# HandBrake/HandBrake

Measured on AMD Instinct MI355X. Metric: filtered frames/sec, 1080p YUV420p NLMeans+decomb chain, higher is better.
Workload: dtype u8 (f32 NLMeans weights, 16-bit fixed-point scaler as zimg, sharpen mix = the reference's f64 expression, as one f32 multiply where init proves that equal); 1 GPU; BASELINE configs[3]: decomb(31, EEDI2 bob) -> nlmeans medium -> cropscale lanczos 1920x1080 -> 3840x2160 -> lapsharp, 1080i YUV420P 8-bit in, inputs resident in HBM; input=1920x1080, output=3840x2160, streams_per_gpu=1, content=interlaced, stream_frames=48, stage_streams=2, parallelism=1 GPU(s) x 1 independent stream(s), device=AMD Radeon Graphics (gfx950:sramecc+:xnack-, 256 CUs)

## Files before the change

### handbrake_amd/csrc/nlmeans.hip

```cpp
#include "hbhip_internal.h"

#include <algorithm>
#include <type_traits>
#include <unordered_map>

namespace {

constexpr int PX = 4;
constexpr int RY = 8;
constexpr int TXN = 32;
constexpr int TYN = 8;
constexpr int TH = TYN * RY;
constexpr int NLM_BORDER = 16;
#ifndef NLM16_SYM_PAIRS
#define NLM16_SYM_PAIRS 3
#endif

struct alignas(16) NlmJob
{
    const uint8_t *frame[HBHIP_NLMEANS_FRAMES_MAX];
    int            fpitch[HBHIP_NLMEANS_FRAMES_MAX];
    const uint8_t *frame_pre[HBHIP_NLMEANS_FRAMES_MAX];
    int            ppitch[HBHIP_NLMEANS_FRAMES_MAX];
    const uint8_t *src_pre;
    int            src_pre_pitch;
    uint8_t       *dst;
    const float   *exptable;
    double         origin_tune;
    float          wft;
    int            diff_max;
    int            diff_cap;
    uint32_t       imul4;
    int            ishift;
    int            w, h, dst_pitch;
    int            nframes, r_half;
    int            tiles_x, tile_start;
};

__global__ void job_table_kernel(uint4 *__restrict__ dst, const uint4 *__restrict__ src, int n16)
{
    const int i = blockIdx.x * blockDim.x + threadIdx.x;
    if (i < n16) dst[i] = src[i];
}

struct __attribute__((packed, aligned(1))) u32_unaligned { uint32_t v; };
typedef float f2 __attribute__((ext_vector_type(2)));

__device__ __forceinline__ int reflect(int x, int n)
{
    x = x < 0 ? -1 - x : x;
    x = x >= n ? 2 * n - 1 - x : x;
    return min(max(x, 0), n - 1);
}

__device__ __forceinline__ uint32_t byte_of(uint32_t v, int k) { return (v >> (8 * k)) & 0xffu; }

constexpr int LTXA = TXN - 2;
constexpr int LTW = LTXA * PX;

__device__ __forceinline__ void load_tile_p(uint32_t *lds, int pitch, int dwords, int rows,
                                            const uint8_t *__restrict__ plane, int src_pitch,
                                            int w, int h, int x0, int y0)
{
    int tid = threadIdx.x;
    asm volatile("" : "+v"(tid));
    const int rpp = (TXN * TYN) / dwords;
    const int r0 = (int)(((float)tid + 0.5f) * (1.0f / (float)dwords));
    const int c = tid - r0 * dwords;
    if (r0 >= rpp) return;
    const int x = x0 + 4 * c;
    const bool whole = x >= 0 && x + 3 < w;
    const int o0 = reflect(x, w), o1 = reflect(x + 1, w), o2 = reflect(x + 2, w), o3 = reflect(x + 3, w);
    uint32_t *out = lds + r0 * pitch + c;
    if (y0 >= 0 && y0 + rows <= h && x0 >= 0 && x0 + 4 * dwords <= w)
    {
        const uint8_t *ptr = plane + (size_t)(y0 + r0) * src_pitch + x;
        const size_t step = (size_t)rpp * src_pitch;
#pragma nounroll
        for (int r = r0; r < rows; r += rpp, out += rpp * pitch, ptr += step)
            *out = reinterpret_cast<const u32_unaligned *>(ptr)->v;
        return;
    }
#pragma nounroll
    for (int r = r0; r < rows; r += rpp, out += rpp * pitch)
    {
        const uint8_t *row = plane + (size_t)reflect(y0 + r, h) * src_pitch;
        uint32_t v;
        if (whole)
            v = reinterpret_cast<const u32_unaligned *>(row + x)->v;
        else
            v = (uint32_t)row[o0] | ((uint32_t)row[o1] << 8) | ((uint32_t)row[o2] << 16) | ((uint32_t)row[o3] << 24);
        *out = v;
    }
}

__device__ __forceinline__ uint32_t from_lane_below(uint32_t x)
{
    return (uint32_t)__builtin_amdgcn_update_dpp(0, (int)x, 0x138 , 0xf, 0xf, false);
}
__device__ __forceinline__ uint32_t from_lane_above(uint32_t x)
{
    return (uint32_t)__builtin_amdgcn_update_dpp(0, (int)x, 0x130 , 0xf, 0xf, false);
}

static bool nlm_no_static_lds(const void *kernel)
{
    hipFuncAttributes a;
    memset(&a, 0, sizeof(a));
    if (hipFuncGetAttributes(&a, kernel) != hipSuccess) { (void)hipGetLastError(); return false; }
    return a.sharedSizeBytes == 0;
}

template <int N, int FAST, int CPD, bool PRE>
__global__ __launch_bounds__(TXN * TYN, 3) void nlmeans_lanes_kernel(const NlmJob *__restrict__ jobs, int njobs,
                                                                     int cmp_rows, int rq)
{
    constexpr int NH = N / 2;
    constexpr int ROWS = RY + N - 1;
    constexpr bool INTIDX = FAST >= 2;
    constexpr bool SYM = FAST == 3 && !PRE;
    static_assert(FAST != 3 || N <= 7, "the pairs' sharing reads a neighbouring lane's edge pixel: patch sizes up to 7");
    constexpr int ST_ROWS = RY + 1, ST_SLOT = ST_ROWS * TXN * TYN;
    static_assert(NH <= PX, "patch must not reach past the adjacent lane");
    static_assert(CPD % 8 == 4, "the two tile rows of a wave must sit 32 banks apart");

    extern __shared__ uint32_t smem[];
    const int tile_dwords = CPD * cmp_rows + 4;
    float *s_exp = reinterpret_cast<float *>(smem);
    uint32_t *s_t0 = smem + 128;
    uint32_t *s_tc = s_t0 + tile_dwords;
    uint32_t *s_r0 = PRE ? s_tc + tile_dwords : s_t0;
    uint32_t *s_rc = PRE ? s_r0 + tile_dwords : s_tc;
    uint32_t *s_stash = s_tc;

    int j = 0;
    for (int hi = njobs - 1; j < hi;)
    {
        const int mid = (j + hi + 1) >> 1;
        if ((int)blockIdx.x >= jobs[mid].tile_start) j = mid; else hi = mid - 1;
    }
    const NlmJob &job = jobs[j];
    const int tile = blockIdx.x - job.tile_start;
    const int tile_y = tile / job.tiles_x;
    int tile_x = tile - tile_y * job.tiles_x;
    if (HBHIP_GRID_ROTATE && (job.tiles_x & 1) == 0) { tile_x += tile_y % job.tiles_x; if (tile_x >= job.tiles_x) tile_x -= job.tiles_x; }
    const int tx0 = tile_x * LTW, ty0 = tile_y * TH;
    const int w = job.w, h = job.h;
    const int RH = job.r_half;

    const int tx = threadIdx.x & (TXN - 1);
    const int ty = threadIdx.x / TXN;

    typedef __attribute__((address_space(3))) const float lds_cfloat;
    __builtin_assume(!INTIDX || reinterpret_cast<uintptr_t>((__attribute__((address_space(3))) uint32_t *)smem) == 0);
    if (threadIdx.x < 128) s_exp[threadIdx.x] = job.exptable[threadIdx.x];
    if (PRE)
    {
        load_tile_p(s_t0, CPD, CPD, cmp_rows, job.src_pre, job.src_pre_pitch, w, h,
                    tx0 - PX - 4 * rq, ty0 - NH - RH);
        load_tile_p(s_r0, CPD, CPD, cmp_rows, job.frame[0], job.fpitch[0], w, h,
                    tx0 - PX - 4 * rq, ty0 - NH - RH);
    }
    else
    {
        load_tile_p(s_t0, CPD, CPD, cmp_rows, job.frame[0], job.fpitch[0], w, h,
                    tx0 - PX - 4 * rq, ty0 - NH - RH);
    }
    const int own_off = (ty * RY + RH) * CPD + tx + rq;
    const uint32_t *own = s_t0 + own_off;
    const uint32_t *own_raw = s_r0 + own_off;

    f2 aw[RY][PX / 2], ap[RY][PX / 2];
#pragma unroll
    for (int o = 0; o < RY; o++)
#pragma unroll
        for (int p = 0; p < PX / 2; p++) { aw[o][p] = f2{0.f, 0.f}; ap[o][p] = f2{0.f, 0.f}; }
    const f2 wft2 = {job.wft, job.wft};

    const float wft = job.wft;
    const int diff_max = job.diff_max;
    const int diff_cap = job.diff_cap;
    const uint32_t imul4 = job.imul4;
    const double origin_tune = job.origin_tune;
    const bool wave_live = ty0 + (ty & ~1) * RY < h;

    for (int f = 0; f < job.nframes; f++)
    {
        if (PRE || f > 0)
        {
            __syncthreads();
            if (PRE)
            {
                load_tile_p(s_tc, CPD, CPD, cmp_rows, job.frame_pre[f], job.ppitch[f], w, h,
                            tx0 - PX - 4 * rq, ty0 - NH - RH);
                if (f > 0)
                    load_tile_p(s_rc, CPD, CPD, cmp_rows, job.frame[f], job.fpitch[f], w, h,
                                tx0 - PX - 4 * rq, ty0 - NH - RH);
            }
            else
            {
                load_tile_p(s_tc, CPD, CPD, cmp_rows, job.frame[f], job.fpitch[f], w, h,
                            tx0 - PX - 4 * rq, ty0 - NH - RH);
            }
        }
        __syncthreads();
        if (!wave_live) continue;
        const uint32_t *cmp_tile = (PRE || f > 0) ? s_tc : s_t0;
        const uint32_t *pix_tile = f > 0 ? s_rc : s_r0;

        auto displacement = [&](auto f0c, int dy, int dx) __attribute__((always_inline))
        {
            constexpr bool F0 = decltype(f0c)::value;
            {
                if (f == 0 && dx == 0 && dy == 0)
                {
#pragma unroll
                    for (int o = 0; o < RY; o++)
                    {
                        const uint32_t cpx = own_raw[(o + NH) * CPD];
#pragma unroll
                        for (int p = 0; p < PX; p++)
                        {
                            aw[o][p / 2][p & 1] = (float)((double)aw[o][p / 2][p & 1] + origin_tune);
                            ap[o][p / 2][p & 1] = (float)((double)ap[o][p / 2][p & 1] + origin_tune * (double)(int)byte_of(cpx, p));
                            __builtin_amdgcn_sched_barrier(0);
                        }
                    }
                    return;
                }

                const int s = dx + 4 * rq;
                const int sh = s & 3;
                if (SYM && F0 && (dy > 0 || (dy == 0 && dx > 0)))
                {
                    const uint32_t *st = s_stash + ((-dy + 1) * 3 + (-dx + 1)) * ST_SLOT + dy * (TXN * TYN) + (int)threadIdx.x;
                    const uint32_t *prow = pix_tile + (ty * RY + dy + RH + NH) * CPD + tx + (s >> 2);
#pragma unroll
                    for (int o = 0; o < RY; o++)
                    {
                        const uint32_t w0 = st[o * (TXN * TYN)];
                        uint32_t id4 = w0;
                        if (dx > 0) id4 = __builtin_amdgcn_alignbyte(st[o * (TXN * TYN) + 1], w0, 1);
                        else if (dx < 0) id4 = __builtin_amdgcn_alignbyte(w0, st[o * (TXN * TYN) - 1], 3);
                        const uint32_t pix = __builtin_amdgcn_alignbyte(prow[o * CPD + 1], prow[o * CPD], sh);
                        const uint32_t o0 = (id4 << 2) & 0x1fcu, o1 = (id4 >> 6) & 0x1fcu, o2 = (id4 >> 14) & 0x1fcu, o3 = (id4 >> 22) & 0x1fcu;
                        const f2 wa = {*reinterpret_cast<lds_cfloat *>(o0), *reinterpret_cast<lds_cfloat *>(o1)};
                        const f2 wb = {*reinterpret_cast<lds_cfloat *>(o2), *reinterpret_cast<lds_cfloat *>(o3)};
                        const f2 pa = {(float)(int)byte_of(pix, 0), (float)(int)byte_of(pix, 1)};
                        const f2 pb = {(float)(int)byte_of(pix, 2), (float)(int)byte_of(pix, 3)};
                        aw[o][0] += wa; ap[o][0] += wa * pa;
                        aw[o][1] += wb; ap[o][1] += wb * pb;
                    }
                    return;
                }
                constexpr bool stash_on = SYM && F0;
                const bool extra_row = stash_on && dy < 0;
                uint32_t *stw = s_stash + ((dy + 1) * 3 + (dx + 1)) * ST_SLOT + (int)threadIdx.x;
                const uint32_t *srow = own;
                const uint32_t *crow = cmp_tile + (ty * RY + dy + RH) * CPD + tx + (s >> 2);

                uint32_t C[PX], hist[RY - 1 + (SYM ? 1 : 0)][PX], v[PX];
                uint32_t centre[NH + 1];
                uint32_t pixq = 0;
                f2 wq[PX / 2];
                const uint32_t *prow = pix_tile + (ty * RY + dy + RH + NH) * CPD + tx + (s >> 2);
#pragma unroll
                for (int q = 0; q < PX; q++) C[q] = 0;

                uint32_t a_n = srow[0], b_n0 = crow[0], b_n1 = crow[1];
#pragma unroll
                for (int i = 0; i < ROWS + (SYM ? 1 : 0); i++)
                {
                    if (!(SYM && i == ROWS) || extra_row)
                    {
                    const uint32_t a = a_n;
                    const uint32_t bw = __builtin_amdgcn_alignbyte(b_n1, b_n0, sh);
                    if (i + 1 < ROWS || (SYM && i + 1 == ROWS && extra_row))
                    {
                        a_n = srow[(i + 1) * CPD];
                        b_n0 = crow[(i + 1) * CPD];
                        b_n1 = crow[(i + 1) * CPD + 1];
                    }
                    if (!PRE) centre[i % (NH + 1)] = bw;
#pragma unroll
                    for (int q = 0; q < PX; q++)
                    {
                        const int d = (int)byte_of(a, q) - (int)byte_of(bw, q);
                        C[q] += (uint32_t)(d * d);
                        if (i < RY - 1 + (SYM ? 1 : 0)) hist[i][q] = C[q];
                    }
                    if (i >= N - 1)
                    {
                        const int o = i - (N - 1);
                        uint32_t V[PX], pre[PX + 1], suf[PX + 1];
#pragma unroll
                        for (int q = 0; q < PX; q++) V[q] = o > 0 ? C[q] - hist[o > 0 ? o - 1 : 0][q] : C[q];
                        pre[0] = 0; suf[0] = 0;
#pragma unroll
                        for (int q = 0; q < PX; q++)
                        {
                            pre[q + 1] = pre[q] + V[q];
                            suf[q + 1] = suf[q] + V[PX - 1 - q];
                        }
#pragma unroll
                        for (int p = 0; p < PX; p++)
                        {
                            const int lo = p - NH, hi = p + NH;
// ... 35 lines not shown
                        {
                            const int o = i - (N - 1);
                            pixq = __builtin_amdgcn_alignbyte(prow[o * CPD + 1], prow[o * CPD], sh);
                        }
                        else
                            pixq = centre[(i - NH) % (NH + 1)];
#pragma unroll
                        for (int pp = 0; pp < PX / 2; pp++)
                        {
                            if (INTIDX)
                                wq[pp] = f2{*reinterpret_cast<lds_cfloat *>(offs[2 * pp]), *reinterpret_cast<lds_cfloat *>(offs[2 * pp + 1])};
                            else
                            {
                                int idx[2];
                                if (FAST == 1)
                                {
                                    const f2 fd = {(float)(int)min(v[2 * pp], (uint32_t)diff_cap),
                                                   (float)(int)min(v[2 * pp + 1], (uint32_t)diff_cap)};
                                    const f2 fi = fd * wft2;
                                    idx[0] = (int)fi.x;
                                    idx[1] = (int)fi.y;
                                }
                                else
                                {
#pragma unroll
                                    for (int e = 0; e < 2; e++)
                                    {
                                        const int diff = (int)v[2 * pp + e];
                                        int ix = (int)((float)diff * wft);
                                        ix = diff < diff_max ? ix : 127;
                                        idx[e] = min(ix, 127);
                                    }
                                }
                                wq[pp] = f2{s_exp[idx[0]], s_exp[idx[1]]};
                            }
                        }
                        }
                    }
                    }
                    __builtin_amdgcn_sched_barrier(0);
                }
                {
                    const uint32_t pix = pixq;
#pragma unroll
                    for (int pp = 0; pp < PX / 2; pp++)
                    {
                        const f2 pv = {(float)(int)byte_of(pix, 2 * pp), (float)(int)byte_of(pix, 2 * pp + 1)};
                        aw[RY - 1][pp] += wq[pp];
                        ap[RY - 1][pp] += wq[pp] * pv;
                    }
                }
            }
        };
        for (int dy = -RH; dy <= RH; dy++)
            for (int dx = -RH; dx <= RH; dx++)
            {
                if (SYM && f == 0) displacement(std::true_type{}, dy, dx);
                else displacement(std::false_type{}, dy, dx);
            }
    }

    const int x = tx0 + (tx - 1) * PX;
    if (tx == 0 || tx == TXN - 1 || x >= w) return;
#pragma unroll
    for (int o = 0; o < RY; o++)
    {
        const int y = ty0 + ty * RY + o;
        if (y >= h) break;
        uint32_t packed = 0;
        const uint32_t cpx = own_raw[(o + NH) * CPD];
#pragma unroll
        for (int p = 0; p < PX; p++)
        {
            const float q = ap[o][p / 2][p & 1] / aw[o][p / 2][p & 1];
            uint32_t r = (uint32_t)(int)q & 0xffu;
            if (r == 0) r = byte_of(cpx, p);
            packed |= r << (8 * p);
            __builtin_amdgcn_sched_barrier(0);
        }
        uint8_t *out = job.dst + (size_t)y * job.dst_pitch + x;
        if (x + 3 < w)
        {
            *reinterpret_cast<uint32_t *>(out) = packed;
        }
        else
        {
            for (int p = 0; p < PX && x + p < w; p++) out[p] = (uint8_t)(packed >> (8 * p));
        }
    }
}

__device__ __forceinline__ void load_tile16(uint32_t *lds, int pitch, int dwords, int rows,
                                            const uint8_t *__restrict__ plane, int src_pitch_bytes,
                                            int w, int h, int x0, int y0)
{
    int tid = threadIdx.x;
    asm volatile("" : "+v"(tid));
    const int rpp = (TXN * TYN) / dwords;
    const int r0 = (int)(((float)tid + 0.5f) * (1.0f / (float)dwords));
    const int c = tid - r0 * dwords;
    if (r0 >= rpp) return;
    const int x = x0 + 2 * c;
    const bool whole = x >= 0 && x + 1 < w;
    const int o0 = reflect(x, w), o1 = reflect(x + 1, w);
    uint32_t *out = lds + r0 * pitch + (c >> 1) + (c & 1) * (pitch >> 1);
#pragma nounroll
    for (int r = r0; r < rows; r += rpp, out += rpp * pitch)
    {
        const uint16_t *row = reinterpret_cast<const uint16_t *>(plane + (size_t)reflect(y0 + r, h) * src_pitch_bytes);
        uint32_t v;
        if (whole)
            v = reinterpret_cast<const u32_unaligned *>(row + x)->v;
        else
            v = (uint32_t)row[o0] | ((uint32_t)row[o1] << 16);
        *out = v;
    }
}

__device__ __forceinline__ uint32_t half_of(uint32_t v, int k) { return (v >> (16 * k)) & 0xffffu; }

typedef short nlm_s2 __attribute__((ext_vector_type(2)));
__device__ __forceinline__ uint32_t pk_sub_i16(uint32_t a, uint32_t b)
{
    return __builtin_bit_cast(uint32_t, (nlm_s2)(__builtin_bit_cast(nlm_s2, a) - __builtin_bit_cast(nlm_s2, b)));
}
__device__ __forceinline__ uint32_t sq_acc_lo(uint32_t d, uint32_t c)
{
    uint32_t r;
    asm("v_mad_i32_i16 %0, %1, %1, %2" : "=v"(r) : "v"(d), "v"(c));
    return r;
}
__device__ __forceinline__ uint32_t sq_acc_hi(uint32_t d, uint32_t c)
{
    uint32_t r;
    asm("v_mad_i32_i16 %0, %1, %1, %2 op_sel:[1,1,0,0]" : "=v"(r) : "v"(d), "v"(c));
    return r;
}

template <int N, int FAST, int CPD, bool PRE, int SYM_PAIRS = 4>
__global__ __launch_bounds__(TXN * TYN, 3) void nlmeans_lanes16_kernel(const NlmJob *__restrict__ jobs, int njobs,
                                                                       int cmp_rows, int rq)
{
    constexpr int NH = N / 2;
    constexpr int ROWS = RY + N - 1;
    constexpr bool SYM = FAST == 3 && !PRE;
    static_assert(FAST != 3 || N <= 7, "the pairs' sharing reads a neighbouring lane's edge pixel: patch sizes up to 7");
    constexpr int ST_ROWS = RY + 1, ST_SLOT = ST_ROWS * TXN * TYN;
    static_assert(NH <= PX, "patch must not reach past the adjacent lane");
    static_assert(CPD % 8 == 4, "the two tile rows of a wave must sit 32 banks apart");
    constexpr int H = CPD / 2;

    extern __shared__ uint32_t smem[];
    const int tile_dwords = CPD * cmp_rows + 4;
    float *s_exp = reinterpret_cast<float *>(smem);
    uint32_t *s_t0 = smem + 128;
    uint32_t *s_tc = s_t0 + tile_dwords;
    uint32_t *s_r0 = PRE ? s_tc + tile_dwords : s_t0;
    uint32_t *s_rc = PRE ? s_r0 + tile_dwords : s_tc;
    uint32_t *s_stash = s_tc;
    typedef __attribute__((address_space(3))) const float lds_cfloat;
    __builtin_assume(FAST < 2 || reinterpret_cast<uintptr_t>((__attribute__((address_space(3))) uint32_t *)smem) == 0);

    int j = 0;
    for (int hi = njobs - 1; j < hi;)
    {
        const int mid = (j + hi + 1) >> 1;
        if ((int)blockIdx.x >= jobs[mid].tile_start) j = mid; else hi = mid - 1;
    }
    const NlmJob &job = jobs[j];
    const int tile = blockIdx.x - job.tile_start;
    const int tile_y = tile / job.tiles_x;
    int tile_x = tile - tile_y * job.tiles_x;
    if (HBHIP_GRID_ROTATE && (job.tiles_x & 1) == 0) { tile_x += tile_y % job.tiles_x; if (tile_x >= job.tiles_x) tile_x -= job.tiles_x; }
    const int tx0 = tile_x * LTW, ty0 = tile_y * TH;
    const int w = job.w, h = job.h;
    const int RH = job.r_half;

    const int tx = threadIdx.x & (TXN - 1);
    const int ty = threadIdx.x / TXN;

    if (threadIdx.x < 128) s_exp[threadIdx.x] = job.exptable[threadIdx.x];
    if (PRE)
    {
        load_tile16(s_t0, CPD, CPD, cmp_rows, job.src_pre, job.src_pre_pitch, w, h, tx0 - PX - 4 * rq, ty0 - NH - RH);
        load_tile16(s_r0, CPD, CPD, cmp_rows, job.frame[0], job.fpitch[0], w, h, tx0 - PX - 4 * rq, ty0 - NH - RH);
    }
    else
        load_tile16(s_t0, CPD, CPD, cmp_rows, job.frame[0], job.fpitch[0], w, h, tx0 - PX - 4 * rq, ty0 - NH - RH);
    const int own_off = (ty * RY + RH) * CPD + tx + rq;
    const uint32_t *own = s_t0 + own_off;
    const uint32_t *own_raw = s_r0 + own_off;

    f2 aw[RY][PX / 2], ap[RY][PX / 2];
#pragma unroll
    for (int o = 0; o < RY; o++)
#pragma unroll
        for (int p = 0; p < PX / 2; p++) { aw[o][p] = f2{0.f, 0.f}; ap[o][p] = f2{0.f, 0.f}; }
    const f2 wft2 = {job.wft, job.wft};
    const float wft = job.wft;
    const int diff_max = job.diff_max;
    const int diff_cap = job.diff_cap;
    const uint32_t imul4 = job.imul4;
    const int ishift = job.ishift;
    const double origin_tune = job.origin_tune;
    const bool wave_live = ty0 + (ty & ~1) * RY < h;

    for (int f = 0; f < job.nframes; f++)
    {
        if (PRE || f > 0)
        {
            __syncthreads();
            if (PRE)
            {
                load_tile16(s_tc, CPD, CPD, cmp_rows, job.frame_pre[f], job.ppitch[f], w, h,
                            tx0 - PX - 4 * rq, ty0 - NH - RH);
                if (f > 0)
                    load_tile16(s_rc, CPD, CPD, cmp_rows, job.frame[f], job.fpitch[f], w, h,
                                tx0 - PX - 4 * rq, ty0 - NH - RH);
            }
            else
                load_tile16(s_tc, CPD, CPD, cmp_rows, job.frame[f], job.fpitch[f], w, h,
                            tx0 - PX - 4 * rq, ty0 - NH - RH);
        }
        __syncthreads();
        if (!wave_live) continue;
        const uint32_t *cmp_tile = (PRE || f > 0) ? s_tc : s_t0;
        const uint32_t *pix_tile = f > 0 ? s_rc : s_r0;

        auto displacement = [&](auto f0c, int dy, int dx) __attribute__((always_inline))
        {
            constexpr bool F0 = decltype(f0c)::value;
            if (f == 0 && dx == 0 && dy == 0)
            {
#pragma unroll
                for (int o = 0; o < RY; o++)
                {
                    const uint32_t c0 = own_raw[(o + NH) * CPD], c1 = own_raw[(o + NH) * CPD + H];
#pragma unroll
                    for (int p = 0; p < PX; p++)
                    {
                        const int sv = (int)half_of(p < 2 ? c0 : c1, p & 1);
                        aw[o][p / 2][p & 1] = (float)((double)aw[o][p / 2][p & 1] + origin_tune);
                        ap[o][p / 2][p & 1] = (float)((double)ap[o][p / 2][p & 1] + origin_tune * (double)sv);
                        __builtin_amdgcn_sched_barrier(0);
                    }
                }
                return;
            }

            const int s = dx + 4 * rq;
            const int sh = 2 * (s & 1);
            const int m = s >> 1;
            const int e0 = (m >> 1) + (m & 1) * H, e1 = ((m + 1) >> 1) + ((m + 1) & 1) * H, e2 = ((m + 2) >> 1) + (m & 1) * H;
            const uint32_t *prow = pix_tile + (ty * RY + dy + RH + NH) * CPD + tx;
            const uint32_t *prow0 = prow + e0, *prow1 = prow + e1, *prow2 = prow + e2;
            const bool shared_pair = SYM_PAIRS == 4 || dy != 0;
            if (SYM && F0 && shared_pair && (dy > 0 || (dy == 0 && dx > 0)))
            {
                const uint32_t *st = s_stash + ((-dy + 1) * 3 + (-dx + 1)) * ST_SLOT + dy * (TXN * TYN) + (int)threadIdx.x;
#pragma unroll
                for (int o = 0; o < RY; o++)
                {
                    const uint32_t w0 = st[o * (TXN * TYN)];
                    uint32_t id4 = w0;
                    if (dx > 0) id4 = __builtin_amdgcn_alignbyte(st[o * (TXN * TYN) + 1], w0, 1);
                    else if (dx < 0) id4 = __builtin_amdgcn_alignbyte(w0, st[o * (TXN * TYN) - 1], 3);
                    const uint32_t p0 = prow0[o * CPD], p1 = prow1[o * CPD], p2 = prow2[o * CPD];
                    const uint32_t pix0 = __builtin_amdgcn_alignbyte(p1, p0, sh), pix1 = __builtin_amdgcn_alignbyte(p2, p1, sh);
                    const uint32_t o0 = (id4 << 2) & 0x1fcu, o1 = (id4 >> 6) & 0x1fcu, o2 = (id4 >> 14) & 0x1fcu, o3 = (id4 >> 22) & 0x1fcu;
                    const f2 wa = {*reinterpret_cast<lds_cfloat *>(o0), *reinterpret_cast<lds_cfloat *>(o1)};
                    const f2 wb = {*reinterpret_cast<lds_cfloat *>(o2), *reinterpret_cast<lds_cfloat *>(o3)};
                    const f2 pa = {(float)(int)half_of(pix0, 0), (float)(int)half_of(pix0, 1)};
                    const f2 pb = {(float)(int)half_of(pix1, 0), (float)(int)half_of(pix1, 1)};
                    aw[o][0] += wa; ap[o][0] += wa * pa;
                    aw[o][1] += wb; ap[o][1] += wb * pb;
// ... 678 lines not shown
            if ((type & PF_REDUCE50) && (type & PF_REDUCE25)) { wet = 1; dry = 3; }
            else if (type & PF_REDUCE50)                      { wet = 1; dry = 1; }
            else if (type & PF_REDUCE25)                      { wet = 3; dry = 1; }
            const dim3 grid((w + 63) / 64, (h + 3) / 4), block(256);
#define PF_LAUNCH(NAME, KERNEL, GRID, BLOCK, ...) do { \
                if (in_geo.bps == 2) HBHIP_LAUNCH(ctx, NAME, KERNEL<uint16_t>, GRID, BLOCK, 0, __VA_ARGS__); \
                else                 HBHIP_LAUNCH(ctx, NAME, KERNEL<uint8_t>, GRID, BLOCK, 0, __VA_ARGS__); } while (0)
            PF_LAUNCH("nlmeans_prefilter", nlm_prefilter_kernel, grid, block,
                      (const uint8_t *)pic->plane[c], pic->pitch[c], q->plane[c], q->pitch[c], w, h, type, wet, dry);
            if (type & PF_EDGEBOOST)
            {
                PF_LAUNCH("nlmeans_edge_mask", nlm_edge_mask_kernel, grid, block,
                          (const uint8_t *)pic->plane[c], pic->pitch[c], mask_pic->plane[c], mask_pic->pitch[c], w, h);
                PF_LAUNCH("nlmeans_edge_apply", nlm_edge_apply_kernel, dim3(1), dim3(EB_THREADS),
                          (const uint8_t *)pic->plane[c], pic->pitch[c], mask_pic->plane[c], mask_pic->pitch[c],
                          q->plane[c], q->pitch[c], w, h);
                if (dry > 0)
                    PF_LAUNCH("nlmeans_prefilter_mix", nlm_mix_kernel, grid, block,
                              (const uint8_t *)pic->plane[c], pic->pitch[c], q->plane[c], q->pitch[c], w, h, wet, dry);
            }
#undef PF_LAUNCH
        }
        HBHIP_CHECK(ctx, hipGetLastError());
        return HBHIP_OK;
    }

    int launch_views(const std::vector<View> &ins, int ready, const std::vector<View> &outs)
    {
        int rc = ensure_jobs(ready * 3);
        if (rc != HBHIP_OK) return rc;
        const int total = (int)ins.size();

        std::vector<int> sizes;
        for (int c = 0; c < 3; c++)
            if (!passthru[c] && par.strength[c] != 0 && std::find(sizes.begin(), sizes.end(), par.patch_size[c]) == sizes.end())
                sizes.push_back(par.patch_size[c]);
        std::sort(sizes.begin(), sizes.end());
        for (int n : sizes)
        {
            const bool generic = force_generic || !(n == 3 || n == 5 || n == 7 || n == 9);
            bool any = false, pre = false;
            for (int c = 0; c < 3; c++)
                if (!passthru[c] && par.strength[c] != 0 && par.patch_size[c] == n)
                {
                    any = true;
                    pre |= pf_type[c] != 0;
                }
            if (!any) continue;
            table = (table + 1) % NTABLES;
            if (table_used[table]) HBHIP_CHECK(ctx, hipEventSynchronize(table_ev[table]));
            NlmJob *hj = h_jobs + (size_t)table * jobs_cap;
            NlmJob *dj = d_jobs + (size_t)table * jobs_cap;
            int nj = 0, tiles = 0, max_rh = 0;
            bool all_rh1 = true;
            bool fast = true, fast_int = true;
            for (int t = 0; t < ready; t++)
                for (int c = 0; c < 3; c++)
                {
                    if (passthru[c] || par.strength[c] == 0 || par.patch_size[c] != n) continue;
                    NlmJob &jb = hj[nj++];
                    jb.nframes = std::min(par.nframes[c], total - t);
                    for (int f = 0; f < jb.nframes; f++)
                    {
                        jb.frame[f] = ins[t + f].plane[c];
                        jb.fpitch[f] = ins[t + f].pitch[c];
                        jb.frame_pre[f] = ins[t + f].pre[c];
                        jb.ppitch[f] = ins[t + f].ppitch[c];
                    }
                    const bool latched_raw = ins[t].first || par.nframes[c] < 2;
                    jb.src_pre = latched_raw ? ins[t].plane[c] : ins[t].pre[c];
                    jb.src_pre_pitch = latched_raw ? ins[t].pitch[c] : ins[t].ppitch[c];
                    jb.dst = outs[t].plane[c];
                    jb.exptable = d_exp + 128 * c;
                    jb.origin_tune = par.origin_tune[c];
                    jb.wft = par.weight_fact_table[c];
                    jb.diff_max = par.diff_max[c];
                    jb.diff_cap = diff_cap[c];
                    jb.imul4 = imul4[c];
                    jb.ishift = ishift[c];
                    fast &= diff_cap[c] >= 0;
                    fast_int &= imul4[c] != 0 && (in_geo.bps == 2 || ishift[c] == 0);
                    jb.w = in_geo.pw[c];
                    jb.h = in_geo.ph[c];
                    jb.dst_pitch = outs[t].pitch[c];
                    jb.r_half = (par.range[c] - 1) / 2;
                    jb.tiles_x = generic ? (jb.w + GW - 1) / GW : (jb.w + LTW - 1) / LTW;
                    jb.tile_start = tiles;
                    tiles += jb.tiles_x * (generic ? (jb.h + GH - 1) / GH : (jb.h + TH - 1) / TH);
                    max_rh = std::max(max_rh, jb.r_half);
                    all_rh1 &= jb.r_half == 1;
                }
            if (nj == 0) continue;
            {
                static_assert(sizeof(NlmJob) % 16 == 0, "NlmJob is copied in 16-byte units");
                const int n16 = (int)(sizeof(NlmJob) * nj / 16);
                HBHIP_LAUNCH(ctx, "nlmeans_job_table", job_table_kernel, dim3((n16 + 255) / 256), dim3(256), 0,
                             reinterpret_cast<uint4 *>(dj), reinterpret_cast<const uint4 *>(h_jobs_dev + (size_t)table * jobs_cap), n16);
            }
            HBHIP_CHECK(ctx, hipEventRecord(table_ev[table], ctx->stream));
            table_used[table] = true;
            const int nh = n / 2;
            if (generic)
            {
                const int aw_ = GW + 2 * nh, ah_ = GH + 2 * nh, bw_ = aw_ + 2 * max_rh, bh_ = ah_ + 2 * max_rh;
                const size_t shmem = sizeof(uint32_t) * ah_ * GW + (size_t)in_geo.bps * (((aw_ * ah_ + 1) & ~1) + bw_ * bh_ + 2);
                if (in_geo.bps == 1)
                    HBHIP_LAUNCH(ctx, "nlmeans_plane_generic", nlmeans_generic_kernel<uint8_t>, dim3(tiles), dim3(GW * GH), shmem, dj, nj, n, max_rh, (int)pre);
                else
                    HBHIP_LAUNCH(ctx, "nlmeans_plane_generic", nlmeans_generic_kernel<uint16_t>, dim3(tiles), dim3(GW * GH), shmem, dj, nj, n, max_rh, (int)pre);
                HBHIP_CHECK(ctx, hipGetLastError());
                continue;
            }
            const int cmp_rows = TH + 2 * (nh + max_rh);
            dim3 grid(tiles), block(TXN * TYN);
            const int rq = (max_rh + 3) / 4;
            const bool wide = in_geo.bps == 2;
            const int cpd = wide ? (rq <= 2 ? 76 : 84) : (rq <= 1 ? 36 : 44);
            const bool sym = fast && fast_int && !pre && all_rh1 && n <= 7;
            size_t shmem = sizeof(uint32_t) * (pre ? 4 : 2) * (cpd * cmp_rows + 4) + 512;
            const int sym_slots = wide ? NLM16_SYM_PAIRS : 4;
            if (sym) shmem = 512 + sizeof(uint32_t) * ((size_t)(cpd * cmp_rows + 4) + std::max<size_t>(cpd * cmp_rows + 4, (size_t)sym_slots * (RY + 1) * TXN * TYN));
#define NLM_LAUNCH(KERNEL) do { \
                static const bool lds_free = nlm_no_static_lds((const void *)KERNEL); \
                if ((fast && fast_int) && !lds_free) return ctx->fail(hipErrorInvalidValue, "nlmeans: kernel has static LDS in front of its table"); \
                if (shmem > 65536) \
                    HBHIP_CHECK(ctx, hipFuncSetAttribute((const void *)KERNEL, hipFuncAttributeMaxDynamicSharedMemorySize, (int)shmem)); \
                HBHIP_LAUNCH(ctx, kname, (KERNEL), grid, block, shmem, dj, nj, cmp_rows, rq); \
            } while (0)
#define NLM_GO(NN, FF, CC, PP) NLM_LAUNCH((nlmeans_lanes_kernel<NN, FF, CC, PP>))
#define NLM_PRE(NN, FF, CC) do { if (pre) NLM_GO(NN, FF, CC, true); else NLM_GO(NN, FF, CC, false); } while (0)
#define NLM_16P(NN, FF, PP) do { if (cpd == 76) NLM_LAUNCH((nlmeans_lanes16_kernel<NN, FF, 76, PP>)); \
                                else NLM_LAUNCH((nlmeans_lanes16_kernel<NN, FF, 84, PP>)); } while (0)
#define NLM_16(NN, FF) do { if (pre) NLM_16P(NN, FF, true); else NLM_16P(NN, FF, false); } while (0)
#define NLM_16S(NN) NLM_LAUNCH((nlmeans_lanes16_kernel<NN, (NN <= 7 ? 3 : 2), 76, false, NLM16_SYM_PAIRS>))
#define NLM_VAR(NN) do { const char *kname = "nlmeans_plane_n" #NN; \
                     if (wide) { if (sym && NN <= 7 && cpd == 76) NLM_16S(NN); else if (fast && fast_int) NLM_16(NN, 2); else if (fast) NLM_16(NN, 1); else NLM_16(NN, 0); } \
                     else if (cpd == 36) { if (sym && NN <= 7) NLM_GO(NN, (NN <= 7 ? 3 : 2), 36, false); else if (fast && fast_int) NLM_PRE(NN, 2, 36); else if (fast) NLM_PRE(NN, 1, 36); else NLM_PRE(NN, 0, 36); } \
                     else { if (sym && NN <= 7) NLM_GO(NN, (NN <= 7 ? 3 : 2), 44, false); else if (fast && fast_int) NLM_PRE(NN, 2, 44); else if (fast) NLM_PRE(NN, 1, 44); else NLM_PRE(NN, 0, 44); } } while (0)
            switch (n)
            {
                case 3: NLM_VAR(3); break;
                case 5: NLM_VAR(5); break;
                case 7: NLM_VAR(7); break;
                case 9: NLM_VAR(9); break;
            }
#undef NLM_VAR
#undef NLM_16
#undef NLM_16P
#undef NLM_16S
#undef NLM_PRE
#undef NLM_GO
#undef NLM_LAUNCH
            HBHIP_CHECK(ctx, hipGetLastError());
        }

        for (int t = 0; t < ready; t++)
            for (int c = 0; c < 3; c++)
                if (passthru[c] || par.strength[c] == 0)
                {
                    const int row = in_geo.pw[c] * in_geo.bps;
                    dim3 grid((row / 4 + 255) / 256 + 1, in_geo.ph[c]);
                    HBHIP_LAUNCH(ctx, "nlmeans_copy_plane", copy_plane_kernel, grid, dim3(256), 0,
                                 outs[t].plane[c], outs[t].pitch[c],
                                 (const uint8_t *)(passthru[c] ? ins[t].pre[c] : ins[t].plane[c]),
                                 passthru[c] ? ins[t].ppitch[c] : ins[t].pitch[c], row, in_geo.ph[c]);
                }
        return HBHIP_OK;
    }

    int schedule(bool draining, bool kicked = false)
    {
        int ready = draining ? (int)in.size() : (int)in.size() - (max_frames - 1);
        if (ready <= 0) return HBHIP_OK;
        if (!draining && !kicked && (deferred || ready < batch)) return HBHIP_OK;

        std::vector<DevPicture *> outs(ready, nullptr);
        std::vector<View> vin, vout;
        for (DevPicture *p : in) vin.push_back(view_of(p));
        for (int t = 0; t < ready; t++)
        {
            outs[t] = pool.acquire();
            if (!outs[t])
            {
                for (int k = 0; k < t; k++) pool.release(outs[k]);
                return HBHIP_ERR_NOMEM;
            }
            outs[t]->tag = in[t]->tag;
            vout.push_back(view_of(outs[t]));
        }
        int rc = launch_views(vin, ready, vout);
        if (rc != HBHIP_OK)
        {
            for (DevPicture *o : outs) pool.release(o);
            return rc;
        }
        for (int t = 0; t < ready; t++)
        {
            out.push_back(outs[t]);
            release_input(in.front());
            in.pop_front();
        }
        return HBHIP_OK;
    }
// ... 90 lines not shown
```

Before: 10010 output frames/s.

## Batch NLMeans tile loads, compute job index arithmetically, specialize origin and symmetric walk

In the fast path, the tile loader now issues all of a thread's global loads into registers before writing any of them to LDS. It is unified for 8-bit and 16-bit planes and uses global address-space pointers. When every frame repeats the same per-plane tile counts, the job index is computed by division instead of a binary search over the job table. The exp-table load is overlapped with the tile loads, and a new template variant uses a plain f32 add for the origin weight when origin_tune is 1. The symmetric first-frame walk is hoisted out of the frame loop with a fixed displacement order. Together these add register pressure and template variants, and a host check rejects tiles taller than the unrolled loader supports.

```diff
diff --git a/handbrake_amd/csrc/nlmeans.hip b/handbrake_amd/csrc/nlmeans.hip
--- a/handbrake_amd/csrc/nlmeans.hip
+++ b/handbrake_amd/csrc/nlmeans.hip
@@ -14,6 +14,13 @@
 constexpr int NLM_BORDER = 16;
 #ifndef NLM16_SYM_PAIRS
 #define NLM16_SYM_PAIRS 3
+#endif
+
+#ifndef NLM_JOB_ARITH
+#define NLM_JOB_ARITH 1
+#endif
+#ifndef NLM_ORIGIN_F32
+#define NLM_ORIGIN_F32 1
 #endif
 
 struct alignas(16) NlmJob
@@ -58,38 +65,83 @@
 constexpr int LTXA = TXN - 2;
 constexpr int LTW = LTXA * PX;
 
-__device__ __forceinline__ void load_tile_p(uint32_t *lds, int pitch, int dwords, int rows,
-                                            const uint8_t *__restrict__ plane, int src_pitch,
-                                            int w, int h, int x0, int y0)
-{
+struct NlmTiles { int per_frame, after0, after1, planes; };
+
+__device__ __forceinline__ int job_of_tile(const NlmJob *__restrict__ jobs, int njobs, const NlmTiles &tc, int &tile)
+{
+    const uint32_t b = blockIdx.x;
+    if (tc.per_frame > 0)
+    {
+        const uint32_t fr = b / (uint32_t)tc.per_frame;
+        const int rem = (int)(b - fr * (uint32_t)tc.per_frame);
+        const int pl = (rem >= tc.after0 ? 1 : 0) + (rem >= tc.after1 ? 1 : 0);
+        tile = rem - (pl == 2 ? tc.after1 : pl == 1 ? tc.after0 : 0);
+        return (int)fr * tc.planes + pl;
+    }
+    int j = 0;
+    for (int hi = njobs - 1; j < hi;)
+    {
+        const int mid = (j + hi + 1) >> 1;
+        if ((int)b >= jobs[mid].tile_start) j = mid; else hi = mid - 1;
+    }
+    tile = (int)b - jobs[j].tile_start;
+    return j;
+}
+
+constexpr int nlm_max_rows(int n, bool sym, int max_rh_of_pitch)
+{
+    return TH + 2 * (sym ? n / 2 + 1 : (n / 2 + max_rh_of_pitch < NLM_BORDER ? n / 2 + max_rh_of_pitch : NLM_BORDER));
+}
+
+#define NLM_GLOBAL __attribute__((address_space(1)))
+typedef const NLM_GLOBAL uint8_t *nlm_gbytes;
+typedef const NLM_GLOBAL u32_unaligned *nlm_gdword;
+template <int BPS, int MAXT>
+__device__ __forceinline__ void load_tile(uint32_t *lds, int pitch, int dwords, int rows,
+                                          const uint8_t *__restrict__ plane, int src_pitch,
+                                          int w, int h, int x0, int y0)
+{
+    constexpr int PPD = 4 / BPS;
     int tid = threadIdx.x;
     asm volatile("" : "+v"(tid));
     const int rpp = (TXN * TYN) / dwords;
     const int r0 = (int)(((float)tid + 0.5f) * (1.0f / (float)dwords));
     const int c = tid - r0 * dwords;
     if (r0 >= rpp) return;
-    const int x = x0 + 4 * c;
-    const bool whole = x >= 0 && x + 3 < w;
-    const int o0 = reflect(x, w), o1 = reflect(x + 1, w), o2 = reflect(x + 2, w), o3 = reflect(x + 3, w);
-    uint32_t *out = lds + r0 * pitch + c;
-    if (y0 >= 0 && y0 + rows <= h && x0 >= 0 && x0 + 4 * dwords <= w)
-    {
-        const uint8_t *ptr = plane + (size_t)(y0 + r0) * src_pitch + x;
+    const int x = x0 + PPD * c;
+    uint32_t *out = lds + r0 * pitch + (BPS == 1 ? c : (c >> 1) + (c & 1) * (pitch >> 1));
+    if (y0 >= 0 && y0 + rows <= h && x0 >= 0 && x0 + PPD * dwords <= w)
+    {
+        __builtin_assume(rows >= TH);
+        const nlm_gbytes ptr = (nlm_gbytes)plane + (size_t)(y0 + r0) * src_pitch + (size_t)x * BPS;
         const size_t step = (size_t)rpp * src_pitch;
-#pragma nounroll
-        for (int r = r0; r < rows; r += rpp, out += rpp * pitch, ptr += step)
-            *out = reinterpret_cast<const u32_unaligned *>(ptr)->v;
+        uint32_t v[MAXT];
+#pragma unroll
+        for (int k = 0; k < MAXT; k++)
+            if (k * rpp < rows && r0 + k * rpp < rows) v[k] = ((nlm_gdword)(ptr + k * step))->v;
+#pragma unroll
+        for (int k = 0; k < MAXT; k++)
+            if (k * rpp < rows && r0 + k * rpp < rows) out[k * rpp * pitch] = v[k];
         return;
     }
+    const bool whole = x >= 0 && x + PPD - 1 < w;
+    int o[PPD];
+#pragma unroll
+    for (int i = 0; i < PPD; i++) o[i] = reflect(x + i, w);
 #pragma nounroll
     for (int r = r0; r < rows; r += rpp, out += rpp * pitch)
     {
-        const uint8_t *row = plane + (size_t)reflect(y0 + r, h) * src_pitch;
+        const nlm_gbytes row = (nlm_gbytes)plane + (size_t)reflect(y0 + r, h) * src_pitch;
         uint32_t v;
         if (whole)
-            v = reinterpret_cast<const u32_unaligned *>(row + x)->v;
+            v = ((nlm_gdword)(row + (size_t)x * BPS))->v;
         else
-            v = (uint32_t)row[o0] | ((uint32_t)row[o1] << 8) | ((uint32_t)row[o2] << 16) | ((uint32_t)row[o3] << 24);
+        {
+            v = 0;
+#pragma unroll
+            for (int i = 0; i < PPD; i++)
+                v |= (BPS == 1 ? (uint32_t)row[o[i]] : (uint32_t)((const NLM_GLOBAL uint16_t *)row)[o[i]]) << (8 * BPS * i);
+        }
         *out = v;
     }
 }
@@ -111,14 +163,15 @@
     return a.sharedSizeBytes == 0;
 }
 
-template <int N, int FAST, int CPD, bool PRE>
+template <int N, int FAST, int CPD, bool PRE, bool ORG1 = false>
 __global__ __launch_bounds__(TXN * TYN, 3) void nlmeans_lanes_kernel(const NlmJob *__restrict__ jobs, int njobs,
-                                                                     int cmp_rows, int rq)
+                                                                     int cmp_rows, int rq, NlmTiles tc)
 {
     constexpr int NH = N / 2;
     constexpr int ROWS = RY + N - 1;
     constexpr bool INTIDX = FAST >= 2;
     constexpr bool SYM = FAST == 3 && !PRE;
+    constexpr int MAXT = (nlm_max_rows(N, SYM, CPD == 36 ? 4 : NLM_BORDER) + (TXN * TYN) / CPD - 1) / ((TXN * TYN) / CPD);
     static_assert(FAST != 3 || N <= 7, "the pairs' sharing reads a neighbouring lane's edge pixel: patch sizes up to 7");
     constexpr int ST_ROWS = RY + 1, ST_SLOT = ST_ROWS * TXN * TYN;
     static_assert(NH <= PX, "patch must not reach past the adjacent lane");
@@ -133,14 +186,8 @@
     uint32_t *s_rc = PRE ? s_r0 + tile_dwords : s_tc;
     uint32_t *s_stash = s_tc;
 
-    int j = 0;
-    for (int hi = njobs - 1; j < hi;)
-    {
-        const int mid = (j + hi + 1) >> 1;
-        if ((int)blockIdx.x >= jobs[mid].tile_start) j = mid; else hi = mid - 1;
-    }
-    const NlmJob &job = jobs[j];
-    const int tile = blockIdx.x - job.tile_start;
+    int tile;
+    const NlmJob &job = jobs[job_of_tile(jobs, njobs, tc, tile)];
     const int tile_y = tile / job.tiles_x;
     int tile_x = tile - tile_y * job.tiles_x;
     if (HBHIP_GRID_ROTATE && (job.tiles_x & 1) == 0) { tile_x += tile_y % job.tiles_x; if (tile_x >= job.tiles_x) tile_x -= job.tiles_x; }
@@ -153,19 +200,21 @@
 
     typedef __attribute__((address_space(3))) const float lds_cfloat;
     __builtin_assume(!INTIDX || reinterpret_cast<uintptr_t>((__attribute__((address_space(3))) uint32_t *)smem) == 0);
-    if (threadIdx.x < 128) s_exp[threadIdx.x] = job.exptable[threadIdx.x];
+    float exp_entry = 0.f;
+    if (threadIdx.x < 128) exp_entry = ((const NLM_GLOBAL float *)job.exptable)[threadIdx.x];
+    const int wx0 = tx0 - PX - 4 * rq, wy0 = ty0 - NH - RH;
+    auto stage = [&](uint32_t *lds, const uint8_t *plane, int pitch) __attribute__((always_inline))
+    {
+        load_tile<1, MAXT>(lds, CPD, CPD, cmp_rows, plane, pitch, w, h, wx0, wy0);
+    };
     if (PRE)
     {
-        load_tile_p(s_t0, CPD, CPD, cmp_rows, job.src_pre, job.src_pre_pitch, w, h,
-                    tx0 - PX - 4 * rq, ty0 - NH - RH);
-        load_tile_p(s_r0, CPD, CPD, cmp_rows, job.frame[0], job.fpitch[0], w, h,
-                    tx0 - PX - 4 * rq, ty0 - NH - RH);
+        stage(s_t0, job.src_pre, job.src_pre_pitch);
+        stage(s_r0, job.frame[0], job.fpitch[0]);
     }
     else
-    {
-        load_tile_p(s_t0, CPD, CPD, cmp_rows, job.frame[0], job.fpitch[0], w, h,
-                    tx0 - PX - 4 * rq, ty0 - NH - RH);
-    }
+        stage(s_t0, job.frame[0], job.fpitch[0]);
+    if (threadIdx.x < 128) s_exp[threadIdx.x] = exp_entry;
     const int own_off = (ty * RY + RH) * CPD + tx + rq;
     const uint32_t *own = s_t0 + own_off;
     const uint32_t *own_raw = s_r0 + own_off;
@@ -184,33 +233,37 @@
     const double origin_tune = job.origin_tune;
     const bool wave_live = ty0 + (ty & ~1) * RY < h;
 
-    for (int f = 0; f < job.nframes; f++)
-    {
-        if (PRE || f > 0)
-        {
-            __syncthreads();
-            if (PRE)
-            {
-                load_tile_p(s_tc, CPD, CPD, cmp_rows, job.frame_pre[f], job.ppitch[f], w, h,
-                            tx0 - PX - 4 * rq, ty0 - NH - RH);
-                if (f > 0)
-                    load_tile_p(s_rc, CPD, CPD, cmp_rows, job.frame[f], job.fpitch[f], w, h,
-                                tx0 - PX - 4 * rq, ty0 - NH - RH);
-            }
-            else
-            {
-                load_tile_p(s_tc, CPD, CPD, cmp_rows, job.frame[f], job.fpitch[f], w, h,
-                            tx0 - PX - 4 * rq, ty0 - NH - RH);
-            }
-        }
-        __syncthreads();
-        if (!wave_live) continue;
+    auto walks = [&](auto f0c, int f) __attribute__((always_inline))
+    {
         const uint32_t *cmp_tile = (PRE || f > 0) ? s_tc : s_t0;
         const uint32_t *pix_tile = f > 0 ? s_rc : s_r0;
 
-        auto displacement = [&](auto f0c, int dy, int dx) __attribute__((always_inline))
-        {
-            constexpr bool F0 = decltype(f0c)::value;
+        auto second = [&](int dy, int dx) __attribute__((always_inline))
+        {
+            const int s = dx + 4 * rq;
+            const int sh = s & 3;
+            const uint32_t *st = s_stash + ((-dy + 1) * 3 + (-dx + 1)) * ST_SLOT + dy * (TXN * TYN) + (int)threadIdx.x;
+            const uint32_t *prow = pix_tile + (ty * RY + dy + RH + NH) * CPD + tx + (s >> 2);
+#pragma unroll
+            for (int o = 0; o < RY; o++)
+            {
+                const uint32_t w0 = st[o * (TXN * TYN)];
+                uint32_t id4 = w0;
+                if (dx > 0) id4 = __builtin_amdgcn_alignbyte(st[o * (TXN * TYN) + 1], w0, 1);
+                else if (dx < 0) id4 = __builtin_amdgcn_alignbyte(w0, st[o * (TXN * TYN) - 1], 3);
+                const uint32_t pix = __builtin_amdgcn_alignbyte(prow[o * CPD + 1], prow[o * CPD], sh);
+                const uint32_t o0 = (id4 << 2) & 0x1fcu, o1 = (id4 >> 6) & 0x1fcu, o2 = (id4 >> 14) & 0x1fcu, o3 = (id4 >> 22) & 0x1fcu;
+                const f2 wa = {*reinterpret_cast<lds_cfloat *>(o0), *reinterpret_cast<lds_cfloat *>(o1)};
+                const f2 wb = {*reinterpret_cast<lds_cfloat *>(o2), *reinterpret_cast<lds_cfloat *>(o3)};
+                const f2 pa = {(float)(int)byte_of(pix, 0), (float)(int)byte_of(pix, 1)};
+                const f2 pb = {(float)(int)byte_of(pix, 2), (float)(int)byte_of(pix, 3)};
+                aw[o][0] += wa; ap[o][0] += wa * pa;
+                aw[o][1] += wb; ap[o][1] += wb * pb;
+            }
+        };
+        auto displacement = [&](auto f0c_, int dy, int dx) __attribute__((always_inline))
+        {
+            constexpr bool F0 = decltype(f0c_)::value;
             {
                 if (f == 0 && dx == 0 && dy == 0)
                 {
@@ -221,6 +274,12 @@
 #pragma unroll
                         for (int p = 0; p < PX; p++)
                         {
+                            if (ORG1)
+                            {
+                                aw[o][p / 2][p & 1] = aw[o][p / 2][p & 1] + 1.0f;
+                                ap[o][p / 2][p & 1] = ap[o][p / 2][p & 1] + (float)(int)byte_of(cpx, p);
+                                continue;
+                            }
                             aw[o][p / 2][p & 1] = (float)((double)aw[o][p / 2][p & 1] + origin_tune);
                             ap[o][p / 2][p & 1] = (float)((double)ap[o][p / 2][p & 1] + origin_tune * (double)(int)byte_of(cpx, p));
                             __builtin_amdgcn_sched_barrier(0);
@@ -231,28 +290,6 @@
 
                 const int s = dx + 4 * rq;
                 const int sh = s & 3;
-                if (SYM && F0 && (dy > 0 || (dy == 0 && dx > 0)))
-                {
-                    const uint32_t *st = s_stash + ((-dy + 1) * 3 + (-dx + 1)) * ST_SLOT + dy * (TXN * TYN) + (int)threadIdx.x;
-                    const uint32_t *prow = pix_tile + (ty * RY + dy + RH + NH) * CPD + tx + (s >> 2);
-#pragma unroll
-                    for (int o = 0; o < RY; o++)
-                    {
-                        const uint32_t w0 = st[o * (TXN * TYN)];
-                        uint32_t id4 = w0;
-                        if (dx > 0) id4 = __builtin_amdgcn_alignbyte(st[o * (TXN * TYN) + 1], w0, 1);
-                        else if (dx < 0) id4 = __builtin_amdgcn_alignbyte(w0, st[o * (TXN * TYN) - 1], 3);
-                        const uint32_t pix = __builtin_amdgcn_alignbyte(prow[o * CPD + 1], prow[o * CPD], sh);
-                        const uint32_t o0 = (id4 << 2) & 0x1fcu, o1 = (id4 >> 6) & 0x1fcu, o2 = (id4 >> 14) & 0x1fcu, o3 = (id4 >> 22) & 0x1fcu;
-                        const f2 wa = {*reinterpret_cast<lds_cfloat *>(o0), *reinterpret_cast<lds_cfloat *>(o1)};
-                        const f2 wb = {*reinterpret_cast<lds_cfloat *>(o2), *reinterpret_cast<lds_cfloat *>(o3)};
-                        const f2 pa = {(float)(int)byte_of(pix, 0), (float)(int)byte_of(pix, 1)};
-                        const f2 pb = {(float)(int)byte_of(pix, 2), (float)(int)byte_of(pix, 3)};
-                        aw[o][0] += wa; ap[o][0] += wa * pa;
-                        aw[o][1] += wb; ap[o][1] += wb * pb;
-                    }
-                    return;
-                }
                 constexpr bool stash_on = SYM && F0;
                 const bool extra_row = stash_on && dy < 0;
                 uint32_t *stw = s_stash + ((dy + 1) * 3 + (dx + 1)) * ST_SLOT + (int)threadIdx.x;
@@ -394,12 +431,38 @@
                 }
             }
         };
-        for (int dy = -RH; dy <= RH; dy++)
-            for (int dx = -RH; dx <= RH; dx++)
-            {
-                if (SYM && f == 0) displacement(std::true_type{}, dy, dx);
-                else displacement(std::false_type{}, dy, dx);
-            }
+        if constexpr (SYM && decltype(f0c)::value)
+        {
+            for (int i = 0; i < 5; i++) displacement(f0c, i < 3 ? -1 : 0, i < 3 ? i - 1 : i - 4);
+            for (int i = 5; i < 9; i++) second(i < 6 ? 0 : 1, i < 6 ? 1 : i - 7);
+        }
+        else
+        {
+            for (int dy = -RH; dy <= RH; dy++)
+                for (int dx = -RH; dx <= RH; dx++) displacement(f0c, dy, dx);
+        }
+    };
+
+    if constexpr (SYM)
+    {
+        __syncthreads();
+        if (wave_live) walks(std::true_type{}, 0);
+    }
+    for (int f = SYM ? 1 : 0; f < job.nframes; f++)
+    {
+        if (PRE || f > 0)
+        {
+            __syncthreads();
+            if (PRE)
+            {
+                stage(s_tc, job.frame_pre[f], job.ppitch[f]);
+                if (f > 0) stage(s_rc, job.frame[f], job.fpitch[f]);
+            }
+            else
+                stage(s_tc, job.frame[f], job.fpitch[f]);
+        }
+        __syncthreads();
+        if (wave_live) walks(std::false_type{}, f);
     }
 
     const int x = tx0 + (tx - 1) * PX;
@@ -432,33 +495,6 @@
     }
 }
 
-__device__ __forceinline__ void load_tile16(uint32_t *lds, int pitch, int dwords, int rows,
-                                            const uint8_t *__restrict__ plane, int src_pitch_bytes,
-                                            int w, int h, int x0, int y0)
-{
-    int tid = threadIdx.x;
-    asm volatile("" : "+v"(tid));
-    const int rpp = (TXN * TYN) / dwords;
-    const int r0 = (int)(((float)tid + 0.5f) * (1.0f / (float)dwords));
-    const int c = tid - r0 * dwords;
-    if (r0 >= rpp) return;
-    const int x = x0 + 2 * c;
-    const bool whole = x >= 0 && x + 1 < w;
-    const int o0 = reflect(x, w), o1 = reflect(x + 1, w);
-    uint32_t *out = lds + r0 * pitch + (c >> 1) + (c & 1) * (pitch >> 1);
-#pragma nounroll
-    for (int r = r0; r < rows; r += rpp, out += rpp * pitch)
-    {
-        const uint16_t *row = reinterpret_cast<const uint16_t *>(plane + (size_t)reflect(y0 + r, h) * src_pitch_bytes);
-        uint32_t v;
-        if (whole)
-            v = reinterpret_cast<const u32_unaligned *>(row + x)->v;
-        else
-            v = (uint32_t)row[o0] | ((uint32_t)row[o1] << 16);
-        *out = v;
-    }
-}
-
 __device__ __forceinline__ uint32_t half_of(uint32_t v, int k) { return (v >> (16 * k)) & 0xffffu; }
 
 typedef short nlm_s2 __attribute__((ext_vector_type(2)));
@@ -481,11 +517,12 @@
 
 template <int N, int FAST, int CPD, bool PRE, int SYM_PAIRS = 4>
 __global__ __launch_bounds__(TXN * TYN, 3) void nlmeans_lanes16_kernel(const NlmJob *__restrict__ jobs, int njobs,
-                                                                       int cmp_rows, int rq)
+                                                                       int cmp_rows, int rq, NlmTiles tc)
 {
     constexpr int NH = N / 2;
     constexpr int ROWS = RY + N - 1;
     constexpr bool SYM = FAST == 3 && !PRE;
+    constexpr int MAXT = (nlm_max_rows(N, SYM, CPD == 76 ? 8 : NLM_BORDER) + (TXN * TYN) / CPD - 1) / ((TXN * TYN) / CPD);
     static_assert(FAST != 3 || N <= 7, "the pairs' sharing reads a neighbouring lane's edge pixel: patch sizes up to 7");
     constexpr int ST_ROWS = RY + 1, ST_SLOT = ST_ROWS * TXN * TYN;
     static_assert(NH <= PX, "patch must not reach past the adjacent lane");
@@ -503,14 +540,8 @@
     typedef __attribute__((address_space(3))) const float lds_cfloat;
     __builtin_assume(FAST < 2 || reinterpret_cast<uintptr_t>((__attribute__((address_space(3))) uint32_t *)smem) == 0);
 
-    int j = 0;
-    for (int hi = njobs - 1; j < hi;)
-    {
-        const int mid = (j + hi + 1) >> 1;
-        if ((int)blockIdx.x >= jobs[mid].tile_start) j = mid; else hi = mid - 1;
-    }
-    const NlmJob &job = jobs[j];
-    const int tile = blockIdx.x - job.tile_start;
+    int tile;
+    const NlmJob &job = jobs[job_of_tile(jobs, njobs, tc, tile)];
     const int tile_y = tile / job.tiles_x;
     int tile_x = tile - tile_y * job.tiles_x;
     if (HBHIP_GRID_ROTATE && (job.tiles_x & 1) == 0) { tile_x += tile_y % job.tiles_x; if (tile_x >= job.tiles_x) tile_x -= job.tiles_x; }
@@ -521,14 +552,20 @@
     const int tx = threadIdx.x & (TXN - 1);
     const int ty = threadIdx.x / TXN;
 
-    if (threadIdx.x < 128) s_exp[threadIdx.x] = job.exptable[threadIdx.x];
+    float exp_entry = 0.f;
+    if (threadIdx.x < 128) exp_entry = ((const NLM_GLOBAL float *)job.exptable)[threadIdx.x];
+    auto stage = [&](uint32_t *lds, const uint8_t *plane, int pitch) __attribute__((always_inline))
+    {
+        load_tile<2, MAXT>(lds, CPD, CPD, cmp_rows, plane, pitch, w, h, tx0 - PX - 4 * rq, ty0 - NH - RH);
+    };
     if (PRE)
     {
-        load_tile16(s_t0, CPD, CPD, cmp_rows, job.src_pre, job.src_pre_pitch, w, h, tx0 - PX - 4 * rq, ty0 - NH - RH);
-        load_tile16(s_r0, CPD, CPD, cmp_rows, job.frame[0], job.fpitch[0], w, h, tx0 - PX - 4 * rq, ty0 - NH - RH);
+        stage(s_t0, job.src_pre, job.src_pre_pitch);
+        stage(s_r0, job.frame[0], job.fpitch[0]);
     }
     else
-        load_tile16(s_t0, CPD, CPD, cmp_rows, job.frame[0], job.fpitch[0], w, h, tx0 - PX - 4 * rq, ty0 - NH - RH);
+        stage(s_t0, job.frame[0], job.fpitch[0]);
+    if (threadIdx.x < 128) s_exp[threadIdx.x] = exp_entry;
     const int own_off = (ty * RY + RH) * CPD + tx + rq;
     const uint32_t *own = s_t0 + own_off;
     const uint32_t *own_raw = s_r0 + own_off;
@@ -554,15 +591,11 @@
             __syncthreads();
             if (PRE)
             {
-                load_tile16(s_tc, CPD, CPD, cmp_rows, job.frame_pre[f], job.ppitch[f], w, h,
-                            tx0 - PX - 4 * rq, ty0 - NH - RH);
-                if (f > 0)
-                    load_tile16(s_rc, CPD, CPD, cmp_rows, job.frame[f], job.fpitch[f], w, h,
-                                tx0 - PX - 4 * rq, ty0 - NH - RH);
+                stage(s_tc, job.frame_pre[f], job.ppitch[f]);
+                if (f > 0) stage(s_rc, job.frame[f], job.fpitch[f]);
             }
             else
-                load_tile16(s_tc, CPD, CPD, cmp_rows, job.frame[f], job.fpitch[f], w, h,
-                            tx0 - PX - 4 * rq, ty0 - NH - RH);
+                stage(s_tc, job.frame[f], job.fpitch[f]);
         }
         __syncthreads();
         if (!wave_live) continue;
@@ -1347,7 +1380,9 @@
             NlmJob *hj = h_jobs + (size_t)table * jobs_cap;
             NlmJob *dj = d_jobs + (size_t)table * jobs_cap;
             int nj = 0, tiles = 0, max_rh = 0;
-            bool all_rh1 = true;
+            bool all_rh1 = true, all_org1 = true;
+            int plane_tiles[3] = {0, 0, 0}, planes = 0;
+            bool repeats = true;
             bool fast = true, fast_int = true;
             for (int t = 0; t < ready; t++)
                 for (int c = 0; c < 3; c++)
@@ -1381,11 +1416,24 @@
                     jb.r_half = (par.range[c] - 1) / 2;
                     jb.tiles_x = generic ? (jb.w + GW - 1) / GW : (jb.w + LTW - 1) / LTW;
                     jb.tile_start = tiles;
-                    tiles += jb.tiles_x * (generic ? (jb.h + GH - 1) / GH : (jb.h + TH - 1) / TH);
+                    const int job_tiles = jb.tiles_x * (generic ? (jb.h + GH - 1) / GH : (jb.h + TH - 1) / TH);
+                    tiles += job_tiles;
+                    if (t == 0) plane_tiles[planes++] = job_tiles;
+                    else repeats &= plane_tiles[(nj - 1) % planes] == job_tiles;
                     max_rh = std::max(max_rh, jb.r_half);
                     all_rh1 &= jb.r_half == 1;
+                    all_org1 &= par.origin_tune[c] == 1.0;
                 }
             if (nj == 0) continue;
+            repeats &= nj == planes * ready;
+            NlmTiles tc = {0, 0, 0, 0};
+            if (repeats && NLM_JOB_ARITH)
+            {
+                tc.per_frame = plane_tiles[0] + plane_tiles[1] + plane_tiles[2];
+                tc.after0 = plane_tiles[0];
+                tc.after1 = plane_tiles[0] + plane_tiles[1];
+                tc.planes = planes;
+            }
             {
                 static_assert(sizeof(NlmJob) % 16 == 0, "NlmJob is copied in 16-byte units");
                 const int n16 = (int)(sizeof(NlmJob) * nj / 16);
@@ -1412,6 +1460,8 @@
             const bool wide = in_geo.bps == 2;
             const int cpd = wide ? (rq <= 2 ? 76 : 84) : (rq <= 1 ? 36 : 44);
             const bool sym = fast && fast_int && !pre && all_rh1 && n <= 7;
+            if (cmp_rows > nlm_max_rows(n, sym, cpd == (wide ? 76 : 36) ? (wide ? 8 : 4) : NLM_BORDER))
+                return ctx->fail(hipErrorInvalidValue, "nlmeans: tile taller than its kernel stages");
             size_t shmem = sizeof(uint32_t) * (pre ? 4 : 2) * (cpd * cmp_rows + 4) + 512;
             const int sym_slots = wide ? NLM16_SYM_PAIRS : 4;
             if (sym) shmem = 512 + sizeof(uint32_t) * ((size_t)(cpd * cmp_rows + 4) + std::max<size_t>(cpd * cmp_rows + 4, (size_t)sym_slots * (RY + 1) * TXN * TYN));
@@ -1420,9 +1470,11 @@
                 if ((fast && fast_int) && !lds_free) return ctx->fail(hipErrorInvalidValue, "nlmeans: kernel has static LDS in front of its table"); \
                 if (shmem > 65536) \
                     HBHIP_CHECK(ctx, hipFuncSetAttribute((const void *)KERNEL, hipFuncAttributeMaxDynamicSharedMemorySize, (int)shmem)); \
-                HBHIP_LAUNCH(ctx, kname, (KERNEL), grid, block, shmem, dj, nj, cmp_rows, rq); \
+                HBHIP_LAUNCH(ctx, kname, (KERNEL), grid, block, shmem, dj, nj, cmp_rows, rq, tc); \
             } while (0)
 #define NLM_GO(NN, FF, CC, PP) NLM_LAUNCH((nlmeans_lanes_kernel<NN, FF, CC, PP>))
+#define NLM_SYM(NN, CC) do { if (all_org1 && NLM_ORIGIN_F32) NLM_LAUNCH((nlmeans_lanes_kernel<NN, (NN <= 7 ? 3 : 2), CC, false, true>)); \
+                             else NLM_GO(NN, (NN <= 7 ? 3 : 2), CC, false); } while (0)
 #define NLM_PRE(NN, FF, CC) do { if (pre) NLM_GO(NN, FF, CC, true); else NLM_GO(NN, FF, CC, false); } while (0)
 #define NLM_16P(NN, FF, PP) do { if (cpd == 76) NLM_LAUNCH((nlmeans_lanes16_kernel<NN, FF, 76, PP>)); \
                                 else NLM_LAUNCH((nlmeans_lanes16_kernel<NN, FF, 84, PP>)); } while (0)
@@ -1430,8 +1482,8 @@
 #define NLM_16S(NN) NLM_LAUNCH((nlmeans_lanes16_kernel<NN, (NN <= 7 ? 3 : 2), 76, false, NLM16_SYM_PAIRS>))
 #define NLM_VAR(NN) do { const char *kname = "nlmeans_plane_n" #NN; \
                      if (wide) { if (sym && NN <= 7 && cpd == 76) NLM_16S(NN); else if (fast && fast_int) NLM_16(NN, 2); else if (fast) NLM_16(NN, 1); else NLM_16(NN, 0); } \
-                     else if (cpd == 36) { if (sym && NN <= 7) NLM_GO(NN, (NN <= 7 ? 3 : 2), 36, false); else if (fast && fast_int) NLM_PRE(NN, 2, 36); else if (fast) NLM_PRE(NN, 1, 36); else NLM_PRE(NN, 0, 36); } \
-                     else { if (sym && NN <= 7) NLM_GO(NN, (NN <= 7 ? 3 : 2), 44, false); else if (fast && fast_int) NLM_PRE(NN, 2, 44); else if (fast) NLM_PRE(NN, 1, 44); else NLM_PRE(NN, 0, 44); } } while (0)
+                     else if (cpd == 36) { if (sym && NN <= 7) NLM_SYM(NN, 36); else if (fast && fast_int) NLM_PRE(NN, 2, 36); else if (fast) NLM_PRE(NN, 1, 36); else NLM_PRE(NN, 0, 36); } \
+                     else { if (sym && NN <= 7) NLM_SYM(NN, 44); else if (fast && fast_int) NLM_PRE(NN, 2, 44); else if (fast) NLM_PRE(NN, 1, 44); else NLM_PRE(NN, 0, 44); } } while (0)
             switch (n)
             {
                 case 3: NLM_VAR(3); break;
@@ -1444,6 +1496,7 @@
 #undef NLM_16P
 #undef NLM_16S
 #undef NLM_PRE
+#undef NLM_SYM
 #undef NLM_GO
 #undef NLM_LAUNCH
             HBHIP_CHECK(ctx, hipGetLastError());
```

After: 10280 output frames/s (median of 6 runs). +2.7%, better.
